# UM-ARM-Lab/pytorch_volumetric

Measured on AMD Instinct MI355X. Metric: SDF (val+grad) queries/sec, higher is better.
Workload: dtype f32

## Files before the change

### pytorch_volumetric_amd/csrc/composed.hip

```cpp
#include "common.h"
#include "grid_lookup.h"
#include "wave_ops.h"
#include "morton.h"

namespace pvamd {

constexpr int kUnnormalised = 1 << 30;
struct Best {
    float v, gx, gy, gz;
    int tag;
};

enum IndexMode { kEstimate = 0, kInlineExact = 1, kExact = 2 };

template <int MODE>
PVAMD_DEV void leaf_candidate(const pvamd_grid_t& g, const float* __restrict__ M, float px, float py, float pz,
                               float& v, float& a, float& b, float& c, uint64_t& vmask, bool& unsure) {
    const float x = affine_row(M[0], M[1], M[2], M[3], px, py, pz);
    const float y = affine_row(M[4], M[5], M[6], M[7], px, py, pz);
    const float z = affine_row(M[8], M[9], M[10], M[11], px, py, pz);
    vmask = in_range_mask(g, x, y, z);
    const bool valid = __builtin_amdgcn_inverse_ballot_w64(vmask);
    auto gather = [&]() {
        int flat;
// ... 901 lines not shown
    constexpr int N = NW * kTilePoints;
    __shared__ __attribute__((aligned(16))) float res[NW][1024];
    __shared__ float cull[kMaxCullLeaves][8];
    const int lane = threadIdx.x & 63, wave = __builtin_amdgcn_readfirstlane(threadIdx.x >> 6);
    const int a = a0 + blockIdx.x;
    build_cull_spheres(grids, S, tf, A, a, cull);
    __syncthreads();
    float scene = __builtin_inff();
    if (S <= kMaxCullLeaves) {
        float reach = -__builtin_inff();
        if (lane < S) {
            const float dx = cull[lane][0] - cull[0][0], dy = cull[lane][1] - cull[0][1], dz = cull[lane][2] - cull[0][2];
            reach = fast_sqrt(dx * dx + dy * dy + dz * dz) + cull[lane][3];
        }
        scene = wave_max(reach);
    }
    const float span = PVAMD_GROUP_MASK_SPAN * scene;
    for (int64_t chunk = blockIdx.y; chunk < nchunks; chunk += gridDim.y) {
        const int64_t cfirst = chunk * N <= P - N ? chunk * N : P - N;
        const int64_t run = chunk * N + wave * kTilePoints;
        const float* tb = bounds + 8 * (chunk * NW + wave);
        const float ct[3] = {tb[0], tb[1], tb[2]};
        const float rt = tb[3], mag = tb[4];
        float lower = -__builtin_inff();
        uint64_t todo = S >= 64 ? ~0ull : ((1ull << S) - 1ull);
        const bool masked = 2.f * rt <= span;
        if (masked) todo = leaf_mask_of_sphere(cull, S, lane, ct, rt, mag, lower);
        const GroupIO gio{sorted + 3 * run, perm + run, &res[0][0], cfirst, nullptr};
        if (masked) tile_passes_split<PPP, false, true, 1>(grids, S, tf, A, a, 0, P, val, leaf, nullptr, lane, todo, lower, gio);
        else tile_passes_split<PPP, false, false, 1>(grids, S, tf, A, a, 0, P, val, leaf, nullptr, lane, todo, lower, gio);
        __syncthreads();
        const f32x4_alias* sp = reinterpret_cast<const f32x4_alias*>(res[wave]);
        const int64_t o = (int64_t)a * P + cfirst + wave * kTilePoints;
        if constexpr (PACKED) {
            const float* rf = res[wave];
            f32x4* rec = reinterpret_cast<f32x4*>(val) + o;
#pragma unroll
            for (int k = 0; k < 4; ++k) {
                const int p = lane + 64 * k;
                rec[p] = f32x4{rf[768 + p], rf[3 * p], rf[3 * p + 1], rf[3 * p + 2]};
            }
        } else {
            __builtin_nontemporal_store(sp[192 + lane], reinterpret_cast<f32x4_u*>(val + o) + lane);
            f32x4_u* dst = reinterpret_cast<f32x4_u*>(grad + 3 * o);
            __builtin_nontemporal_store(sp[lane], dst + lane);
            __builtin_nontemporal_store(sp[lane + 64], dst + lane + 64);
            __builtin_nontemporal_store(sp[lane + 128], dst + lane + 128);
        }
        __syncthreads();
    }
}


template <int NW, int PPP>
__global__ __launch_bounds__(NW * 64, PVAMD_GROUP_MINWAVES) void composed_query_fused(
    const pvamd_grid_t* __restrict__ grids, int S, const float* __restrict__ tf, int A, const float* __restrict__ pts, int64_t nchunks,
    int64_t P, float* __restrict__ val, float* __restrict__ grad, int* __restrict__ leaf, int a0) {
    constexpr int N = NW * kTilePoints, kBins = N < 4096 ? N : 4096, kPerThread = kBins / (NW * 64), kKeyShift = kBins == 4096 ? 0 : (kBins == 2048 ? 1 : 2);
    static_assert(kBins >= 1024 && kBins % (NW * 64) == 0, "4, 8 or 16 waves");
    __shared__ __attribute__((aligned(16))) float res[NW][1024];
    __shared__ uint16_t sperm[N];
    __shared__ unsigned box[6];
    __shared__ unsigned wsum[NW];
    __shared__ __attribute__((aligned(16))) float wspan[NW];
    const int lane = threadIdx.x & 63, wave = __builtin_amdgcn_readfirstlane(threadIdx.x >> 6);
    const int a = a0 + blockIdx.x;
    auto hist = [&](int bin) -> unsigned& { return reinterpret_cast<unsigned*>(res[bin >> 8])[768 + (bin & 255)]; };
    for (int64_t chunk = blockIdx.y; chunk < nchunks; chunk += gridDim.y) {
        const int64_t cfirst = chunk * N <= P - N ? chunk * N : P - N;
        f32x4_alias* sp = reinterpret_cast<f32x4_alias*>(res[wave]);
        {
            const f32x4_u* src = reinterpret_cast<const f32x4_u*>(pts + 3 * (cfirst + wave * kTilePoints));
            sp[lane] = src[lane];
            sp[lane + 64] = src[lane + 64];
            sp[lane + 128] = src[lane + 128];
        }
        for (int i = threadIdx.x; i < kBins; i += NW * 64) hist(i) = 0u;
        if (threadIdx.x < 3) {
            box[threadIdx.x] = 0xffffffffu;
            box[3 + threadIdx.x] = 0u;
        }
        PVAMD_WAVE_SYNC();
        const f32x4 q0 = sp[3 * lane], q1 = sp[3 * lane + 1], q2 = sp[3 * lane + 2];
        const float px[4] = {q0.x, q0.w, q1.z, q2.y}, py[4] = {q0.y, q1.x, q1.w, q2.z}, pz[4] = {q0.z, q1.y, q2.x, q2.w};
        float lo[3], hi[3];
#pragma unroll
        for (int d = 0; d < 3; ++d) {
            lo[d] = __builtin_inff();
            hi[d] = -__builtin_inff();
        }
#pragma unroll
        for (int k = 0; k < 4; ++k) {
            const float c[3] = {px[k], py[k], pz[k]};
#pragma unroll
            for (int d = 0; d < 3; ++d) {
                const bool fin = fabsf(c[d]) < __builtin_inff();
                lo[d] = fin ? fminf(lo[d], c[d]) : lo[d];
                hi[d] = fin ? fmaxf(hi[d], c[d]) : hi[d];
            }
        }
        __syncthreads();
        float tile_span = 0.f;
#pragma unroll
        for (int d = 0; d < 3; ++d) {
            const float l = wave_min(lo[d]), h = wave_max(hi[d]);
            tile_span += fmaxf(h - l, 0.f);
            if (lane == 0) {
                atomicMin(&box[d], order_code(l));
                atomicMax(&box[3 + d], order_code(h));
            }
        }
        if (lane == 0) wspan[wave] = tile_span;
        __syncthreads();
        float blo[3], scale[3], chunk_span = 0.f;
#pragma unroll
        for (int d = 0; d < 3; ++d) {
            blo[d] = order_decode(box[d]);
            const float ext = order_decode(box[3 + d]) - blo[d];
            chunk_span += fmaxf(ext, 0.f);
            scale[d] = 15.999f / fmaxf(ext, 1e-30f);
        }
        float worst_tile = 0.f;
        if constexpr (NW % 4 == 0) {
            const f32x4_alias* w4 = reinterpret_cast<const f32x4_alias*>(wspan);
#pragma unroll
            for (int w = 0; w < NW / 4; ++w) {
                const f32x4 v = w4[w];
                worst_tile = fmaxf(worst_tile, fmaxf(fmaxf(v.x, v.y), fmaxf(v.z, v.w)));
            }
        } else {
            for (int w = 0; w < NW; ++w) worst_tile = fmaxf(worst_tile, wspan[w]);
        }
        const bool coherent = worst_tile <= kCoherentSpan * chunk_span;
        if (coherent) {
#pragma unroll
            for (int k = 0; k < 4; ++k) sperm[wave * kTilePoints + 4 * lane + k] = (uint16_t)(wave * kTilePoints + 4 * lane + k);
            PVAMD_WAVE_SYNC();
        } else {
        unsigned key[4], rank[4];
#pragma unroll
        for (int k = 0; k < 4; ++k) {
            key[k] = hilbert_cell16(px[k], py[k], pz[k], blo, scale) >> kKeyShift;
            rank[k] = atomicAdd(&hist((int)key[k]), 1u);
        }
        __syncthreads();
        unsigned local[kPerThread], sum = 0u;
#pragma unroll
        for (int i = 0; i < kPerThread; ++i) {
            local[i] = hist((int)threadIdx.x * kPerThread + i);
            sum += local[i];
        }
        unsigned inc = sum;
#pragma unroll
        for (int off = 1; off < 64; off <<= 1) {
            const unsigned t = __shfl_up(inc, off);
            inc += lane >= off ? t : 0u;
        }
        if (lane == 63) wsum[wave] = inc;
        __syncthreads();
        unsigned base = inc - sum;
        for (int w = 0; w < wave; ++w) base += wsum[w];
#pragma unroll
        for (int i = 0; i < kPerThread; ++i) {
            hist((int)threadIdx.x * kPerThread + i) = base;
            base += local[i];
        }
        __syncthreads();
#pragma unroll
        for (int k = 0; k < 4; ++k) sperm[hist((int)key[k]) + rank[k]] = (uint16_t)(wave * kTilePoints + 4 * lane + k);
        __syncthreads();
        }
        const GroupIO gio{nullptr, nullptr, &res[0][0], cfirst, sperm + wave * kTilePoints};
        const uint64_t todo = S >= 64 ? ~0ull : ((1ull << S) - 1ull);
        tile_passes_split<PPP, false, false, 2>(grids, S, tf, A, a, 0, P, val, leaf, nullptr, lane, todo, -__builtin_inff(), gio);
        __syncthreads();
        const int64_t o = (int64_t)a * P + cfirst + wave * kTilePoints;
        __builtin_nontemporal_store(sp[192 + lane], reinterpret_cast<f32x4_u*>(val + o) + lane);
        f32x4_u* dst = reinterpret_cast<f32x4_u*>(grad + 3 * o);
        __builtin_nontemporal_store(sp[lane], dst + lane);
        __builtin_nontemporal_store(sp[lane + 64], dst + lane + 64);
        __builtin_nontemporal_store(sp[lane + 128], dst + lane + 128);
        __syncthreads();
    }
}

}

using namespace pvamd;

static inline bool legacy_leaf_loop(int32_t flags, int32_t S) { return (flags & PVAMD_COMPOSED_LEGACY_LEAF_LOOP) || S >= kNoLeaf; }

extern "C" int pvamd_composed_query_packed(const pvamd_grid_t* grids, int32_t S, const float* tf, int32_t A,
                                           const float* points, int64_t Pp, float* out_rec, int32_t flags, void* stream) {
    if (S < 1 || A < 1 || Pp < 1 || Pp % kTilePoints != 0 || S >= kUnnormalised) return PVAMD_E_SHAPE;
    if (!grids || !tf || !points || !out_rec) return PVAMD_E_NULL;
    if (!aligned_to(grids, 8) || !aligned_to(tf, 4) || !aligned_to(points, 16) || !aligned_to(out_rec, 16)) return PVAMD_E_ALIGN;
    hipStream_t s = (hipStream_t)stream;
    const int64_t ntiles = Pp / kTilePoints;
    const int64_t tile_blocks = (ntiles + kWavesPerBlock - 1) / kWavesPerBlock;
    if (tile_blocks > 65535) return PVAMD_E_SHAPE;
    if (flags & PVAMD_COMPOSED_INLINE_EXACT)
        hipLaunchKernelGGL((composed_query_wave<PVAMD_COMPOSED_PPP, kInlineExact, true, 0>), dim3(A, (unsigned)tile_blocks),
                           dim3(kWavesPerBlock * 64), 0, s, grids, S, tf, A, points, ntiles, Pp, out_rec, nullptr, nullptr, 0);
    else if (legacy_leaf_loop(flags, S))
        hipLaunchKernelGGL((composed_query_wave<PVAMD_COMPOSED_PPP, kEstimate, true, 0>), dim3(A, (unsigned)tile_blocks),
                           dim3(kWavesPerBlock * 64), 0, s, grids, S, tf, A, points, ntiles, Pp, out_rec, nullptr, nullptr, 0);
    else
        hipLaunchKernelGGL((composed_query_wave<PVAMD_COMPOSED_PPP, kEstimate, true, 1>), dim3(A, (unsigned)tile_blocks),
                           dim3(kWavesPerBlock * 64), 0, s, grids, S, tf, A, points, ntiles, Pp, out_rec, nullptr, nullptr, 0);
    return (int)hipGetLastError();
}

extern "C" int pvamd_unpack_records(const float* rec, const int32_t* index, int64_t P, int64_t stride, int32_t A,
                                    float* out_val, float* out_grad, void* stream) {
    if (A < 1 || P < 1 || stride < 1) return PVAMD_E_SHAPE;
    if (!rec || !index || !out_val || !out_grad) return PVAMD_E_NULL;
    if (!aligned_to(rec, 16) || !aligned_to(index, 4) || !aligned_to(out_val, 4) || !aligned_to(out_grad, 4)) return PVAMD_E_ALIGN;
    const int64_t ntiles = (P + kTilePoints - 1) / kTilePoints;
    const int64_t tile_blocks = (ntiles + kUnpermuteWaves - 1) / kUnpermuteWaves;
    const int64_t groups = ((int64_t)A + 7) / 8;
    const int64_t ublocks = (tile_blocks + kUnpermuteTiles - 1) / kUnpermuteTiles;
    const int64_t blocks = groups * 8 * ublocks;
// ... 148 lines not shown
```

### pytorch_volumetric_amd/csrc/mesh.hip

```cpp
#include <cstdlib>
#include "common.h"
#include "mesh_math.h"
#include "morton.h"
#include "order_small.h"
#include "wave_ops.h"

namespace pvamd {

constexpr int kRec = PVAMD_TRI_REC;
constexpr int kTile = PVAMD_TRI_TILE;
constexpr int kGroup = PVAMD_TRI_GROUP;
constexpr int kGroupsPerTile = kTile / kGroup;
static_assert(kTile == 256 && kGroup == 16 && kRec == 24, "the scan is written for 256-record tiles of six float4 planes");
enum { kPlaneSphere = 0, kPlaneU = 1, kPlaneV = 2, kPlaneA = 3, kPlaneB = 4, kPlaneC = 5 };
constexpr int kTileFloats = kTile * kRec;
PVAMD_DEV const f32x4* tile_plane(const float* rec, int tile, int plane) {
    return reinterpret_cast<const f32x4*>(rec + (int64_t)tile * kTileFloats + plane * (kTile * 4));
}
PVAMD_DEV f32x4 record_plane(const float* rec, int j, int plane) { return tile_plane(rec, j / kTile, plane)[j % kTile]; }

struct MeshArgs {
    const float* normal;
    const float* rec;
    const float* tiles;
// ... 158 lines not shown
    const float du = fmaxf(fabsf(u) - hu, 0.f), dv = fmaxf(fabsf(v) - hv, 0.f);
    const float lb2 = fmaf(dv, dv, fmaf(du, du, h2));
    return !(lb2 > fmaf(8e-6f, dist2, s.reach2m + m0));
}

#ifdef PVAMD_MESH_STATS
__device__ unsigned long long g_stats[32];
__device__ long long g_nested;
#define STAT(i, v) do { if ((threadIdx.x & 63) == 0) atomicAdd(&g_stats[i], (unsigned long long)(v)); } while (0)
extern "C" int pvamd_debug_stats(unsigned long long* out, int reset) {
    (void)hipMemcpyFromSymbol(out, HIP_SYMBOL(g_stats), sizeof(g_stats));
    if (reset) { unsigned long long z[32] = {}; (void)hipMemcpyToSymbol(HIP_SYMBOL(g_stats), z, sizeof(z)); }
    return 0;
}
#define TIC(t) const long long t = __builtin_readcyclecounter()
#define TOC(i, t) STAT(i, __builtin_readcyclecounter() - t)
#define TOC_NET(i, t, inner) STAT(i, __builtin_readcyclecounter() - t - (inner))
#else
#define STAT(i, v)
#define TIC(t)
#define TOC(i, t)
#define TOC_NET(i, t, inner)
#endif

constexpr int kQueueCap = 128;
constexpr unsigned long long kBestInit = 0x7F80000000000000ull;

template <bool WITH_RAY>
struct WaveLocal {
    f32x4 sphere[64], fu[64], fv[64];
    float m0[64];
    unsigned qc[kQueueCap];
    unsigned qr[WITH_RAY ? kQueueCap : 1];
};
template <bool WITH_RAY>
struct GroupShared {
    unsigned long long best[64];
    int hits[WITH_RAY ? 64 : 1];
    int handed;
    float dir[WITH_RAY ? 192 : 1];
    float dn[WITH_RAY ? 192 : 1];
};
template <int SLICES, bool WITH_RAY>
struct MeshShared {
    GroupShared<WITH_RAY> g;
    WaveLocal<WITH_RAY> w[SLICES];
};

PVAMD_DEV float uniform(float v) { return __int_as_float(__builtin_amdgcn_readfirstlane(__float_as_int(v))); }
PVAMD_DEV V3 xyz(f32x4 v) { return v3(v.x, v.y, v.z); }

struct WaveBound {
    LaneState q;
    float rho;
    V3 dn0;
    float k, rho_k;
};

template <bool WITH_RAY>
struct Wave {
    LaneState s;
    bool live;
    V3 dn, dir;
    WaveBound wb;
    int nc, nr;
};

template <bool WITH_RAY>
PVAMD_DEV void refresh_bound(Wave<WITH_RAY>& wv) {
    const float rmax = wave_max(wv.live ? wv.s.reach : 0.f);
    set_reach(wv.wb.q, uniform((rmax + wv.wb.rho) * 1.00001f));
}

template <bool WITH_RAY>
PVAMD_DEV void pull_reach(const GroupShared<WITH_RAY>& g, Wave<WITH_RAY>& wv) {
    const float d2 = __int_as_float((int)(unsigned)(g.best[threadIdx.x & 63] >> 32));
    const float reach = fast_sqrt(d2) * 1.00001f + 1.1e-19f;
    if (reach < wv.s.reach) set_reach(wv.s, reach);
    refresh_bound(wv);
}

template <bool WITH_RAY>
PVAMD_DEV bool wave_setup(const MeshArgs& m, Wave<WITH_RAY>& wv) {
    const V3 p = wv.s.p;
    wv.live = fabsf(p.x) < INFINITY && fabsf(p.y) < INFINITY && fabsf(p.z) < INFINITY;
    wv.nc = wv.nr = 0;
    set_reach(wv.s, INFINITY);
    if (__ballot(wv.live) == 0ull) return false;
    const float lx = wave_min(wv.live ? p.x : INFINITY), hx = wave_max(wv.live ? p.x : -INFINITY);
    const float ly = wave_min(wv.live ? p.y : INFINITY), hy = wave_max(wv.live ? p.y : -INFINITY);
    const float lz = wave_min(wv.live ? p.z : INFINITY), hz = wave_max(wv.live ? p.z : -INFINITY);
    wv.wb.q.p = v3(uniform(0.5f * lx + 0.5f * hx), uniform(0.5f * ly + 0.5f * hy), uniform(0.5f * lz + 0.5f * hz));
    const V3 d = v3(p.x - wv.wb.q.p.x, p.y - wv.wb.q.p.y, p.z - wv.wb.q.p.z);
    wv.wb.rho = uniform(wave_max(wv.live ? fast_sqrt(dot(d, d)) : 0.f) * 1.00001f + 1.1e-19f);
    wv.wb.dn0 = v3(0.f, 0.f, 0.f);
    wv.wb.k = wv.wb.rho_k = 0.f;
    if (WITH_RAY) {
        const V3 a = v3((float)m.ray_dir[0], (float)m.ray_dir[1], (float)m.ray_dir[2]);
        const float inv = 1.f / sqrt_rn(dot(a, a));
        wv.wb.dn0 = v3(uniform(a.x * inv), uniform(a.y * inv), uniform(a.z * inv));
        const V3 e = v3(wv.dn.x - wv.wb.dn0.x, wv.dn.y - wv.wb.dn0.y, wv.dn.z - wv.wb.dn0.z);
        const float chord = wave_max(wv.live ? fast_sqrt(dot(e, e)) : 0.f);
        wv.wb.k = uniform(2.001f * chord + 2e-6f);
        wv.wb.rho_k = uniform(wv.wb.rho * (1.f + wv.wb.k) * 1.00001f);
    }
    set_reach(wv.wb.q, INFINITY);
    return true;
}

PVAMD_DEV bool axis_may_hit(const WaveBound& wb, V3 w, float dist2, float r) {
    const float dist = fast_sqrt(dist2) * 1.00001f + 1.1e-19f;
    return sphere_may_hit(dist2, dot(w, wb.dn0), fmaf(wb.k, dist, r + wb.rho_k));
}

PVAMD_DEV void enqueue(unsigned* q, int& n, unsigned long long mask, bool mine, int j) {
    const int lane = threadIdx.x & 63;
    if (mine) q[n + __popcll(mask & ((1ull << lane) - 1ull))] = ((unsigned)j << 6) | (unsigned)lane;
    n += __popcll(mask);
}

template <class Fn>
PVAMD_DEV void drain(unsigned* q, int& n, bool everything, Fn&& fn) {
    const int lane = threadIdx.x & 63;
    PVAMD_WAVE_SYNC();
    STAT(6, 1);
    fn(n < 64 ? n : 64, q);
    if (n > 64) {
        const int rem = n - 64;
        if (everything) {
            STAT(6, 1);
            fn(rem, q + 64);
            n = 0;
        } else {
            const unsigned v = lane < rem ? q[64 + lane] : 0u;
            if (lane < rem) q[lane] = v;
            n = rem;
        }
    } else {
        n = 0;
    }
    PVAMD_WAVE_SYNC();
}

template <bool WITH_RAY>
PVAMD_DEV void drain_closest(const MeshArgs& m, GroupShared<WITH_RAY>& g, WaveLocal<WITH_RAY>& wl, Wave<WITH_RAY>& wv, bool everything) {
    if (wv.nc == 0) return;
    const int lane = threadIdx.x & 63;
    TIC(t_drain);
    drain(wl.qc, wv.nc, everything, [&](int count, const unsigned* q) {
        PVAMD_COUNT_PAIRS(m, 0, count);
        const unsigned e = lane < count ? q[lane] : 0u;
        const int owner = e & 63;
        const V3 p = v3(__shfl(wv.s.p.x, owner, 64), __shfl(wv.s.p.y, owner, 64), __shfl(wv.s.p.z, owner, 64));
        if (lane < count) {
            const int j = (int)(e >> 6);
            const f32x4 A = record_plane(m.rec, j, kPlaneA), B = record_plane(m.rec, j, kPlaneB), C = record_plane(m.rec, j, kPlaneC);
            const V3 qp = sub(closest_point_triangle(p, xyz(A), xyz(B), xyz(C)), p);
            const float d2 = dot(qp, qp);
            atomicMin(&g.best[owner], ((unsigned long long)(unsigned)__float_as_int(d2) << 32) | (unsigned)__float_as_int(A.w));
        }
    });
    pull_reach(g, wv);
    TOC(16, t_drain);
}

template <bool WITH_RAY>
PVAMD_DEV void drain_rays(const MeshArgs& m, GroupShared<WITH_RAY>& g, WaveLocal<WITH_RAY>& wl, Wave<WITH_RAY>& wv, bool everything) {
    if (wv.nr == 0) return;
    const int lane = threadIdx.x & 63;
    drain(wl.qr, wv.nr, everything, [&](int count, const unsigned* q) {
        PVAMD_COUNT_PAIRS(m, 1, count);
        const unsigned e = lane < count ? q[lane] : 0u;
        const int owner = e & 63;
        const V3 p = v3(__shfl(wv.s.p.x, owner, 64), __shfl(wv.s.p.y, owner, 64), __shfl(wv.s.p.z, owner, 64));
        const V3 d = v3(__shfl(wv.dir.x, owner, 64), __shfl(wv.dir.y, owner, 64), __shfl(wv.dir.z, owner, 64));
        if (lane < count) {
            const int j = (int)(e >> 6);
            const f32x4 A = record_plane(m.rec, j, kPlaneA), B = record_plane(m.rec, j, kPlaneB), C = record_plane(m.rec, j, kPlaneC);
            if (ray_hits_triangle(p, d, xyz(A), xyz(B), xyz(C))) atomicAdd(&g.hits[owner], 1);
        }
    });
}

template <bool WITH_RAY>
PVAMD_DEV void visit_tile(const MeshArgs& m, GroupShared<WITH_RAY>& g, WaveLocal<WITH_RAY>& wl, Wave<WITH_RAY>& wv, int ti,
                          int pass_lo = 0, int pass_hi = kTile / 64) {
    const int lane = threadIdx.x & 63;
    const int ntiles = (m.F + kTile - 1) / kTile;
    const int n = min(kTile, m.F - ti * kTile);
    STAT(1, 1);
    TIC(t_visit);
    unsigned gm = 0u;
#ifdef PVAMD_MESH_STATS
    unsigned mine_groups = 0u;
#endif
    {
        const bool gv = lane < kGroupsPerTile && lane * kGroup < n;
        const f32x4 gs = reinterpret_cast<const f32x4*>(m.tiles)[ntiles + ti * kGroupsPerTile + (gv ? lane : 0)];
        const V3 wc = v3(gs.x - wv.wb.q.p.x, gs.y - wv.wb.q.p.y, gs.z - wv.wb.q.p.z);
        const float dc2 = dot(wc, wc);
        bool coarse = sphere_may_improve(wv.wb.q, dc2, gs.w);
        if (WITH_RAY) coarse = coarse || axis_may_hit(wv.wb, wc, dc2, gs.w);
        unsigned todo = (unsigned)__ballot(coarse && gv);
        todo &= ((1u << (pass_hi * (64 / kGroup))) - 1u) & ~((1u << (pass_lo * (64 / kGroup))) - 1u);
        while (todo != 0u) {
            const int b = __builtin_ctz(todo);
            todo &= todo - 1u;
            const V3 ctr = v3(__int_as_float(__builtin_amdgcn_readlane(__float_as_int(gs.x), b)),
                              __int_as_float(__builtin_amdgcn_readlane(__float_as_int(gs.y), b)),
                              __int_as_float(__builtin_amdgcn_readlane(__float_as_int(gs.z), b)));
            const float r = __int_as_float(__builtin_amdgcn_readlane(__float_as_int(gs.w), b));
            const V3 w = v3(ctr.x - wv.s.p.x, ctr.y - wv.s.p.y, ctr.z - wv.s.p.z);
            const float dist2 = dot(w, w);
            bool need = sphere_may_improve(wv.s, dist2, r);
            if (WITH_RAY) need = need || sphere_may_hit(dist2, dot(w, wv.dn), r);
            STAT(9, 1);
#ifdef PVAMD_MESH_STATS
            if (need && wv.live) mine_groups |= 1u << b;
#endif
            if (__ballot(need && wv.live) != 0ull) gm |= 1u << b;
        }
    }
    const f32x4* P0 = tile_plane(m.rec, ti, kPlaneSphere);
    const f32x4* P1 = tile_plane(m.rec, ti, kPlaneU);
    const f32x4* P2 = tile_plane(m.rec, ti, kPlaneV);
    const f32x4* P4 = tile_plane(m.rec, ti, kPlaneB);
    for (int pass = pass_lo; pass < pass_hi; ++pass) {
        if (((gm >> (pass * (64 / kGroup))) & ((1u << (64 / kGroup)) - 1u)) == 0u) continue;
        STAT(2, 1);
#ifdef PVAMD_MESH_STATS
        {
            const int st_points = __popcll(__ballot(((mine_groups >> (pass * (64 / kGroup))) & 0xFu) != 0u));
            STAT(22, st_points);
        }
#endif
        const int idx = pass * 64 + lane;
        const f32x4 a0 = P0[idx], a1 = P1[idx], a2 = P2[idx];
        const float am0 = P4[idx].w;
        bool keep_c, keep_r = false;
        {
            const bool valid = idx < n && ((gm >> (idx / kGroup)) & 1u);
            const V3 w = v3(a0.x - wv.wb.q.p.x, a0.y - wv.wb.q.p.y, a0.z - wv.wb.q.p.z);
            const float dist2 = dot(w, w);
            keep_c = valid && sphere_may_improve(wv.wb.q, dist2, a0.w) &&
                     rect_may_improve(wv.wb.q, w, dist2, xyz(a1), a1.w, xyz(a2), a2.w, am0);
            if (WITH_RAY) keep_r = valid && axis_may_hit(wv.wb, w, dist2, a0.w);
        }
        const unsigned long long mc = __ballot(keep_c), mr = WITH_RAY ? __ballot(keep_r) : 0ull;
        unsigned long long todo = mc | mr;
        if (todo == 0ull) continue;
        PVAMD_WAVE_SYNC();
        wl.sphere[lane] = a0;
        wl.fu[lane] = a1;
        wl.fv[lane] = a2;
        wl.m0[lane] = am0;
        PVAMD_WAVE_SYNC();
        const int j0 = ti * kTile + pass * 64;
        const unsigned long long live_mask = __ballot(wv.live);
        TIC(t_surv);
        while (todo != 0ull) {
            const int b = __builtin_ctzll(todo);
            todo &= todo - 1ull;
            STAT(3, 1);
            const f32x4 o = wl.sphere[b];
            const V3 w = v3(o.x - wv.s.p.x, o.y - wv.s.p.y, o.z - wv.s.p.z);
            const float dist2 = dot(w, w);
            if (!WITH_RAY || ((mc >> b) & 1ull)) {
                const unsigned long long near_c = live_mask & __ballot(sphere_may_improve(wv.s, dist2, o.w));
                if (near_c != 0ull) {
                    STAT(7, 1);
                    const f32x4 u = wl.fu[b], v = wl.fv[b];
                    const unsigned long long mk = near_c & __ballot(rect_may_improve(wv.s, w, dist2, xyz(u), u.w, xyz(v), v.w, wl.m0[b]));
                    if (mk) {
                        STAT(4, __popcll(mk)); STAT(8, 1);
                        enqueue(wl.qc, wv.nc, mk, __builtin_amdgcn_inverse_ballot_w64(mk), j0 + b);
                        if (wv.nc >= 64) drain_closest(m, g, wl, wv, false);
                    }
                }
            }
            if (WITH_RAY && ((mr >> b) & 1ull)) {
                const unsigned long long mk = live_mask & __ballot(sphere_may_hit(dist2, dot(w, wv.dn), o.w));
                if (mk) {
                    STAT(5, __popcll(mk)); STAT(8, 1);
                    enqueue(wl.qr, wv.nr, mk, __builtin_amdgcn_inverse_ballot_w64(mk), j0 + b);
                    if (wv.nr >= 64) drain_rays(m, g, wl, wv, false);
                }
            }
        }
        TOC(18, t_surv);
    }
    TOC(17, t_visit);
}

template <bool WITH_RAY>
PVAMD_DEV int scan_seed(const MeshArgs& m, Wave<WITH_RAY>& wv, int part, int nparts) {
    const int lane = threadIdx.x & 63;
    const int ntiles = (m.F + kTile - 1) / kTile;
    const f32x4* tiles4 = reinterpret_cast<const f32x4*>(m.tiles);
// ... 9 lines not shown
            if ((nparts == 1 || (ti % nparts) == part) && (b < own || nearest < 0)) {
                own = b < own ? b : own;
                nearest = ti;
            }
        }
    }
    const float lowest = wave_min(bound);
    set_reach(wv.s, (lowest + wv.wb.rho) * 1.00001f);
    refresh_bound(wv);
    const float mine = wave_min(own);
    unsigned long long at = __ballot(nearest >= 0 && own == mine);
    if (at == 0ull) at = __ballot(nearest >= 0);
    return at ? __builtin_amdgcn_readlane(nearest, __builtin_ctzll(at)) : -1;
}

template <bool WITH_RAY>
PVAMD_DEV void greedy_reach(const MeshArgs& m, GroupShared<WITH_RAY>& g, Wave<WITH_RAY>& wv, int ti) {
    const int ntiles = (m.F + kTile - 1) / kTile;
    const f32x4* spheres = reinterpret_cast<const f32x4*>(m.tiles);
    const V3 p = wv.s.p;
    auto reach_of = [&](f32x4 sp) {
        const V3 w = v3(sp.x - p.x, sp.y - p.y, sp.z - p.z);
        return fast_sqrt(dot(w, w)) * 1.00001f + (sp.w + 1.1e-19f);
    };
    float bound = INFINITY;
    int gi = 0;
    const int ngroups = (min(kTile, m.F - ti * kTile) + kGroup - 1) / kGroup;
    for (int k = 0; k < ngroups; ++k) {
        const float b = reach_of(spheres[ntiles + ti * kGroupsPerTile + k]);
        if (b < bound) { bound = b; gi = k; }
    }
    const int j0 = ti * kTile + gi * kGroup;
    float nearest = INFINITY;
    int jn = -1;
    for (int k = 0; k < kGroup; ++k) {
        if (j0 + k < m.F) {
            const float b = reach_of(record_plane(m.rec, j0 + k, kPlaneSphere));
            if (b < nearest) { nearest = b; jn = j0 + k; }
        }
    }
#ifndef PVAMD_MESH_NO_GREEDY_EXACT
    PVAMD_COUNT_PAIRS(m, 0, __popcll(__ballot(jn >= 0 && wv.live)));
    if (jn >= 0 && wv.live) {
        const f32x4 A = record_plane(m.rec, jn, kPlaneA), B = record_plane(m.rec, jn, kPlaneB), C = record_plane(m.rec, jn, kPlaneC);
        const V3 qp = sub(closest_point_triangle(p, xyz(A), xyz(B), xyz(C)), p);
        const float d2 = dot(qp, qp);
        atomicMin(&g.best[threadIdx.x & 63], ((unsigned long long)(unsigned)__float_as_int(d2) << 32) | (unsigned)__float_as_int(A.w));
        STAT(4, 1);
    }
#endif
    bound = fminf(bound, nearest) * 1.00001f;
    if (bound < wv.s.reach) set_reach(wv.s, bound);
    pull_reach(g, wv);
}

template <bool WITH_RAY>
PVAMD_DEV void scan_tiles(const MeshArgs& m, GroupShared<WITH_RAY>& g, WaveLocal<WITH_RAY>& wl, Wave<WITH_RAY>& wv, int skip,
                          int part, int nparts, int pass_lo = 0, int pass_hi = kTile / 64) {
    const int lane = threadIdx.x & 63;
    const int ntiles = (m.F + kTile - 1) / kTile;
    const f32x4* tiles4 = reinterpret_cast<const f32x4*>(m.tiles);
    for (int base = 0; base < ntiles; base += 64) {
        const int ti = base + lane;
        const bool mine = ti < ntiles && ti != skip && (nparts == 1 || (ti % nparts) == part);
        const f32x4 ts = tiles4[mine ? ti : 0];
        const V3 w = v3(ts.x - wv.wb.q.p.x, ts.y - wv.wb.q.p.y, ts.z - wv.wb.q.p.z);
        const float dist2 = dot(w, w);
        const bool ray = WITH_RAY && mine && axis_may_hit(wv.wb, w, dist2, ts.w);
        STAT(0, 1);
        const float lower = mine ? fast_sqrt(dist2) - ts.w : INFINITY;
        unsigned long long done = 0ull;
        for (;;) {
            pull_reach(g, wv);
            const bool need = mine && (ray || sphere_may_improve(wv.wb.q, dist2, ts.w));
            const unsigned long long todo = __ballot(need) & ~done;
            if (todo == 0ull) break;
            const float key = ((todo >> lane) & 1ull) ? lower : INFINITY;
            const unsigned long long at = __ballot(key == wave_min(key)) & todo;
            const int t = __builtin_ctzll(at ? at : todo);
            done |= 1ull << t;
            const V3 ctr = v3(__int_as_float(__builtin_amdgcn_readlane(__float_as_int(ts.x), t)),
                              __int_as_float(__builtin_amdgcn_readlane(__float_as_int(ts.y), t)),
                              __int_as_float(__builtin_amdgcn_readlane(__float_as_int(ts.z), t)));
            const float r = __int_as_float(__builtin_amdgcn_readlane(__float_as_int(ts.w), t));
            const V3 wl_ = v3(ctr.x - wv.s.p.x, ctr.y - wv.s.p.y, ctr.z - wv.s.p.z);
            const float d2 = dot(wl_, wl_);
            bool mine_too = sphere_may_improve(wv.s, d2, r);
            if (WITH_RAY) mine_too = mine_too || sphere_may_hit(d2, dot(wl_, wv.dn), r);
            if (__ballot(mine_too && wv.live) == 0ull) continue;
            visit_tile<WITH_RAY>(m, g, wl, wv, base + t, pass_lo, pass_hi);
        }
    }
}

template <bool WITH_RAY>
PVAMD_DEV void scan_finish(const MeshArgs& m, GroupShared<WITH_RAY>& g, WaveLocal<WITH_RAY>& wl, Wave<WITH_RAY>& wv) {
    drain_closest(m, g, wl, wv, true);
    if (WITH_RAY) drain_rays(m, g, wl, wv, true);
}

template <bool WITH_RAY>
PVAMD_DEV bool scan_begin(const MeshArgs& m, GroupShared<WITH_RAY>& g, Wave<WITH_RAY>& wv, int wave, uint64_t seed,
                          int64_t jitter_index, const unsigned long long* start, const float* __restrict__ drawn = nullptr,
                          const float* __restrict__ bound = nullptr) {
    const int lane = threadIdx.x & 63;
    if (wave == 0) {
        g.best[lane] = start ? *start : kBestInit;
        if (WITH_RAY) {
            g.hits[lane] = 0;
            const V3 dir = drawn ? v3(drawn[3 * lane], drawn[3 * lane + 1], drawn[3 * lane + 2])
                                 : jitter_dir(m.ray_dir, seed, jitter_index);
            const float inv_len = 1.f / sqrt_rn(dot(dir, dir));
            g.dir[3 * lane] = dir.x; g.dir[3 * lane + 1] = dir.y; g.dir[3 * lane + 2] = dir.z;
            g.dn[3 * lane] = dir.x * inv_len; g.dn[3 * lane + 1] = dir.y * inv_len; g.dn[3 * lane + 2] = dir.z * inv_len;
        }
    }
    __syncthreads();
    wv.dir = wv.dn = v3(0.f, 0.f, 0.f);
    if (WITH_RAY) {
        wv.dir = v3(g.dir[3 * lane], g.dir[3 * lane + 1], g.dir[3 * lane + 2]);
        wv.dn = v3(g.dn[3 * lane], g.dn[3 * lane + 1], g.dn[3 * lane + 2]);
    }
    return bound ? load_bound(bound, wv) : wave_setup(m, wv);
}

struct HandOver {
    int* count;
// ... 35 lines not shown
#endif
#ifndef PVAMD_MESH_HEAVY_PARTS
#define PVAMD_MESH_HEAVY_PARTS 32
#endif
constexpr int kHeavy32nds = PVAMD_MESH_HEAVY_32NDS;
#ifndef PVAMD_MESH_HEAVY_MIN_TILES
#define PVAMD_MESH_HEAVY_MIN_TILES 128
#endif
constexpr int kHeavyMinTiles = PVAMD_MESH_HEAVY_MIN_TILES;
constexpr int kHeavyParts = PVAMD_MESH_HEAVY_PARTS;

PVAMD_DEV void store_bound(float* __restrict__ b, const WaveBound& wb, bool any_live) {
    if ((threadIdx.x & 63) != 0) return;
    b[0] = wb.q.p.x; b[1] = wb.q.p.y; b[2] = wb.q.p.z; b[3] = wb.rho;
    b[4] = wb.dn0.x; b[5] = wb.dn0.y; b[6] = wb.dn0.z; b[7] = wb.k;
    b[8] = wb.rho_k; b[9] = any_live ? 1.f : 0.f;
    b[10] = wb.q.reach;
}
template <bool WITH_RAY>
PVAMD_DEV bool part_has_work(const MeshArgs& m, const float* __restrict__ b, int part, int nparts) {
    if (uniform(b[9]) == 0.f) return false;
    WaveBound wb;
    wb.q.p = v3(uniform(b[0]), uniform(b[1]), uniform(b[2]));
    wb.rho = uniform(b[3]);
    wb.dn0 = v3(uniform(b[4]), uniform(b[5]), uniform(b[6]));
    wb.k = uniform(b[7]);
    wb.rho_k = uniform(b[8]);
    set_reach(wb.q, uniform(b[10]));
    const int lane = threadIdx.x & 63;
    const int ntiles = (m.F + kTile - 1) / kTile;
    const f32x4* tiles4 = reinterpret_cast<const f32x4*>(m.tiles);
    for (int base = part; base < ntiles; base += 64 * nparts) {
        const int ti = base + lane * nparts;
        const f32x4 ts = tiles4[ti < ntiles ? ti : 0];
        const V3 w = v3(ts.x - wb.q.p.x, ts.y - wb.q.p.y, ts.z - wb.q.p.z);
        const float dist2 = dot(w, w);
        bool need = sphere_may_improve(wb.q, dist2, ts.w);
        if (WITH_RAY) need = need || axis_may_hit(wb, w, dist2, ts.w);
        if (__ballot(need && ti < ntiles) != 0ull) return true;
    }
    return false;
}
template <bool WITH_RAY>
PVAMD_DEV bool load_bound(const float* __restrict__ b, Wave<WITH_RAY>& wv) {
    const V3 p = wv.s.p;
    wv.live = fabsf(p.x) < INFINITY && fabsf(p.y) < INFINITY && fabsf(p.z) < INFINITY;
    wv.nc = wv.nr = 0;
    set_reach(wv.s, INFINITY);
    wv.wb.q.p = v3(uniform(b[0]), uniform(b[1]), uniform(b[2]));
    wv.wb.rho = uniform(b[3]);
    wv.wb.dn0 = v3(uniform(b[4]), uniform(b[5]), uniform(b[6]));
    wv.wb.k = uniform(b[7]);
    wv.wb.rho_k = uniform(b[8]);
    set_reach(wv.wb.q, INFINITY);
    return uniform(b[9]) != 0.f;
}

template <bool WITH_RAY>
PVAMD_DEV int flagged_tiles(const MeshArgs& m, const Wave<WITH_RAY>& wv) {
    const int lane = threadIdx.x & 63;
    const int ntiles = (m.F + kTile - 1) / kTile;
    const f32x4* tiles4 = reinterpret_cast<const f32x4*>(m.tiles);
    int n = 0;
    for (int base = 0; base < ntiles; base += 64) {
        const int ti = base + lane;
        const f32x4 ts = tiles4[ti < ntiles ? ti : 0];
        const V3 w = v3(ts.x - wv.wb.q.p.x, ts.y - wv.wb.q.p.y, ts.z - wv.wb.q.p.z);
        const float dist2 = dot(w, w);
        bool need = sphere_may_improve(wv.wb.q, dist2, ts.w);
        if (WITH_RAY) need = need || axis_may_hit(wv.wb, w, dist2, ts.w);
        n += __popcll(__ballot(need && ti < ntiles));
    }
    return n;
}

template <int SLICES, bool WITH_RAY>
PVAMD_DEV bool scan_mesh(const MeshArgs& m, MeshShared<SLICES, WITH_RAY>& sh, Wave<WITH_RAY>& wv, int wave, uint64_t seed,
                         int64_t jitter_index, const HandOver& ho, int group, int transform) {
    const int lane = threadIdx.x & 63;
    bool handed = false;
    TIC(t_all);
    if (scan_begin(m, sh.g, wv, wave, seed, jitter_index, nullptr) && m.F > 0) {
        TIC(t_seed);
        const int first = scan_seed(m, wv, wave, SLICES);
        if (first >= 0) {
#ifndef PVAMD_MESH_NO_GREEDY
            greedy_reach(m, sh.g, wv, first);
#endif
            TOC(20, t_seed);
            visit_tile<WITH_RAY>(m, sh.g, sh.w[wave], wv, first);
            drain_closest(m, sh.g, sh.w[wave], wv, true);
        }
        if (ho.cap > 0 && (m.F + kTile - 1) / kTile >= kHeavyMinTiles) {
            __syncthreads();
            if (wave == 0) {
                pull_reach(sh.g, wv);
                int slot = -1;
                if (flagged_tiles(m, wv) * 32 >= ((m.F + kTile - 1) / kTile) * kHeavy32nds) {
                    if (lane == 0) slot = atomicAdd(ho.count, 1);
                    slot = __builtin_amdgcn_readfirstlane(slot);
                    if (slot >= ho.cap) slot = -1;
                }
                if (slot >= 0) {
                    if (lane == 0) {
                        ho.entries[2 * slot] = group;
                        ho.entries[2 * slot + 1] = transform;
// ... 266 lines not shown

__global__ __launch_bounds__(64) void hand_over_gather_kernel(MeshArgs m, const int* __restrict__ order, const float* __restrict__ pts,
                                                              int64_t P, HandOver ho, int groups) {
    const int g = blockIdx.x, lane = threadIdx.x;
    const int64_t slot = (int64_t)g * 64 + lane;
    const int64_t i = point_index(order, slot, P);
    const V3 dir = v3(ho.p_dir[3 * i], ho.p_dir[3 * i + 1], ho.p_dir[3 * i + 2]);
    const float reach = ho.p_reach[i];
    ho.best[slot] = ho.p_best[i];
    ho.reach[slot] = reach;
    ho.hits[slot] = 0;
    float* o = ho.dir + slot * 3;
    o[0] = dir.x; o[1] = dir.y; o[2] = dir.z;
    Wave<true> wv{};
    wv.s.p = v3(pts[3 * i], pts[3 * i + 1], pts[3 * i + 2]);
    float* q = ho.pts + slot * 3;
    q[0] = wv.s.p.x; q[1] = wv.s.p.y; q[2] = wv.s.p.z;
    const float inv_len = 1.f / sqrt_rn(dot(dir, dir));
    wv.dir = dir;
    wv.dn = v3(dir.x * inv_len, dir.y * inv_len, dir.z * inv_len);
    const bool any_live = wave_setup(m, wv);
    if (any_live) {
        set_reach(wv.s, reach);
        refresh_bound(wv);
    }
    store_bound(ho.bound + (int64_t)g * kBoundFloats, wv.wb, any_live);
    if (lane == 0) {
        ho.entries[2 * g] = g;
        ho.entries[2 * g + 1] = 0;
        if (g == 0) *ho.count = groups;
    }
}

#ifndef PVAMD_MESH_PARTS_WAVES
#define PVAMD_MESH_PARTS_WAVES 7
#endif
template <bool WITH_RAY, bool WAIT = false, int WAVES = kTile / 64>
PVAMD_DEV void parts_of_group(const MeshArgs& m, MeshShared<WAVES, WITH_RAY>& sh, const int* __restrict__ order,
                              const float* __restrict__ M, const float* __restrict__ pts, int64_t P, uint64_t seed,
                              int64_t index_base, const HandOver& ho, int slot, int group) {
    const int lane = threadIdx.x & 63, wave = __builtin_amdgcn_readfirstlane(threadIdx.x >> 6);
    if (!part_has_work<WITH_RAY>(m, ho.bound + (int64_t)slot * kBoundFloats, (int)blockIdx.y, (int)gridDim.y)) return;
    Wave<WITH_RAY> wv;
    const float* q = ho.pts + ((int64_t)slot * 64 + lane) * 3;
    wv.s.p = v3(q[0], q[1], q[2]);
    const unsigned long long start = ho.best[(int64_t)slot * 64 + lane];
    const float known = ho.reach[(int64_t)slot * 64 + lane];
    TIC(t_parts);
    if (scan_begin(m, sh.g, wv, wave, seed, 0, &start, WITH_RAY ? ho.dir + (int64_t)slot * 192 : nullptr,
                   ho.bound + (int64_t)slot * kBoundFloats)) {
        if (__any(wv.live && !(known < INFINITY) && (unsigned)(start >> 32) >= 0x7F800000u)) scan_seed(m, wv, 0, 1);
        if (known < wv.s.reach) set_reach(wv.s, known);
        refresh_bound(wv);
        constexpr int kPasses = (kTile / 64) / WAVES;
        scan_tiles<WITH_RAY>(m, sh.g, sh.w[wave], wv, -1, (int)blockIdx.y, (int)gridDim.y, wave * kPasses, (wave + 1) * kPasses);
        scan_finish(m, sh.g, sh.w[wave], wv);
    }
    TOC(21, t_parts);
    __syncthreads();
    if (wave == 0) {
        if (WAIT) {
            unsigned long long was = 0ull;
            int had = 0;
            if (sh.g.best[lane] < start) was = atomicMin(&ho.best[(int64_t)slot * 64 + lane], sh.g.best[lane]);
            if (WITH_RAY && sh.g.hits[lane] != 0) had = atomicAdd(&ho.hits[(int64_t)slot * 64 + lane], sh.g.hits[lane]);
            asm volatile("" ::"v"(was), "v"(had) : "memory");
        } else {
            if (sh.g.best[lane] < start) atomicMin(&ho.best[(int64_t)slot * 64 + lane], sh.g.best[lane]);
            if (WITH_RAY && sh.g.hits[lane] != 0) atomicAdd(&ho.hits[(int64_t)slot * 64 + lane], sh.g.hits[lane]);
        }
    }
}

template <int kAllWaves>
__global__ __launch_bounds__(64 * kAllWaves, PVAMD_MESH_PARTS_WAVES) void mesh_parts_all_kernel(MeshArgs m, const int* __restrict__ order,
                                                                          const float* __restrict__ pts, int64_t P,
                                                                          uint64_t seed, int64_t index_base, HandOver ho, QueryOut out) {
    __shared__ __attribute__((aligned(16))) MeshShared<kAllWaves, true> sh;
    const int g = (int)blockIdx.x;
    parts_of_group<true, true, kAllWaves>(m, sh, order, nullptr, pts, P, seed, index_base, ho, g, g);
    if (threadIdx.x >= 64) return;
    const int lane = threadIdx.x;
    int done = 0;
    if (lane == 0) done = atomicAdd(&ho.entries[2 * g + 1], 1);
    if (__builtin_amdgcn_readfirstlane(done) != (int)gridDim.y - 1) return;
    const int64_t k = (int64_t)g * 64 + lane;
    if (k >= P) return;
    const int64_t i = order ? (int64_t)order[k] : k;
    const unsigned long long found = atomicMin(&ho.best[k], ~0ull);
    const int hits = atomicOr(&ho.hits[k], 0);
    write_query(m, out, i, v3(pts[3 * i], pts[3 * i + 1], pts[3 * i + 2]), found, hits);
}

template <bool WITH_RAY, int WAVES>
__global__ __launch_bounds__(64 * WAVES, PVAMD_MESH_PARTS_WAVES) void mesh_parts_kernel(MeshArgs m, const int* __restrict__ order,
                                                                      const float* __restrict__ W,
                                                                      const float* __restrict__ pts, int64_t P,
                                                                      uint64_t seed, int64_t index_base, HandOver ho) {
    __shared__ __attribute__((aligned(16))) MeshShared<WAVES, WITH_RAY> sh;
    const int listed = min(*ho.count, ho.cap);
    for (int slot = blockIdx.x; slot < listed; slot += gridDim.x) {
        parts_of_group<WITH_RAY, false, WAVES>(m, sh, order, W ? W + 16 * (int64_t)ho.entries[2 * slot + 1] : nullptr, pts, P, seed, index_base,
                                 ho, slot, ho.entries[2 * slot]);
        __syncthreads();
    }
}
// ... 351 lines not shown
```

Baseline: 203.6 billion.

## Shrink fused-kernel sort histogram and replace block scans with wave-local DPP scan

Reduces the Hilbert-key histogram in the fused composed query kernel to a small configurable bin count (default 512) held in its own shared array. Every wave now computes the exclusive prefix redundantly with a DPP inclusive scan, which removes the cross-wave scan, its two block barriers and the per-wave sum array. The chunk bounding box is reduced from per-wave slots with group reductions instead of shared atomics, which also drops one barrier. In exchange the Hilbert ordering is coarser, so the sort may give less spatial coherence for grid lookups. The bin starts are also packed as uint16 into each wave's scratch area.

```diff
diff --git a/pytorch_volumetric_amd/csrc/composed.hip b/pytorch_volumetric_amd/csrc/composed.hip
--- a/pytorch_volumetric_amd/csrc/composed.hip
+++ b/pytorch_volumetric_amd/csrc/composed.hip
@@ -977,20 +977,37 @@
 }
 
 
+#ifndef PVAMD_FUSED_BINS
+#define PVAMD_FUSED_BINS 512
+#endif
+constexpr int kFusedBins = PVAMD_FUSED_BINS;
+typedef unsigned u32_alias __attribute__((may_alias));
+typedef uint16_t u16_alias __attribute__((may_alias));
+
+PVAMD_DEV unsigned wave_inclusive_sum(unsigned v) {
+    v += (unsigned)__builtin_amdgcn_update_dpp(0, (int)v, 0x111, 0xf, 0xf, false);
+    v += (unsigned)__builtin_amdgcn_update_dpp(0, (int)v, 0x112, 0xf, 0xf, false);
+    v += (unsigned)__builtin_amdgcn_update_dpp(0, (int)v, 0x114, 0xf, 0xf, false);
+    v += (unsigned)__builtin_amdgcn_update_dpp(0, (int)v, 0x118, 0xf, 0xf, false);
+    v += (unsigned)__builtin_amdgcn_update_dpp(0, (int)v, 0x142, 0xa, 0xf, false);
+    v += (unsigned)__builtin_amdgcn_update_dpp(0, (int)v, 0x143, 0xc, 0xf, false);
+    return v;
+}
+
 template <int NW, int PPP>
 __global__ __launch_bounds__(NW * 64, PVAMD_GROUP_MINWAVES) void composed_query_fused(
     const pvamd_grid_t* __restrict__ grids, int S, const float* __restrict__ tf, int A, const float* __restrict__ pts, int64_t nchunks,
     int64_t P, float* __restrict__ val, float* __restrict__ grad, int* __restrict__ leaf, int a0) {
-    constexpr int N = NW * kTilePoints, kBins = N < 4096 ? N : 4096, kPerThread = kBins / (NW * 64), kKeyShift = kBins == 4096 ? 0 : (kBins == 2048 ? 1 : 2);
-    static_assert(kBins >= 1024 && kBins % (NW * 64) == 0, "4, 8 or 16 waves");
+    constexpr int N = NW * kTilePoints, kBins = kFusedBins, kPerLane = kBins / 64;
+    constexpr int kKeyShift = kBins == 512 ? 3 : (kBins == 256 ? 4 : (kBins == 128 ? 5 : 6));
+    static_assert(kBins == 512 || kBins == 256 || kBins == 128 || kBins == 64, "a wave's uint16 bin starts fill at most its 1 KB value quarter");
+    static_assert(NW <= 16 && (NW & (NW - 1)) == 0 && N <= 65535, "a row of 16 lanes folds the wave boxes; positions are uint16");
     __shared__ __attribute__((aligned(16))) float res[NW][1024];
     __shared__ uint16_t sperm[N];
-    __shared__ unsigned box[6];
-    __shared__ unsigned wsum[NW];
-    __shared__ __attribute__((aligned(16))) float wspan[NW];
+    __shared__ __attribute__((aligned(16))) unsigned hist[kBins];
+    __shared__ float wbox[7][NW];
     const int lane = threadIdx.x & 63, wave = __builtin_amdgcn_readfirstlane(threadIdx.x >> 6);
     const int a = a0 + blockIdx.x;
-    auto hist = [&](int bin) -> unsigned& { return reinterpret_cast<unsigned*>(res[bin >> 8])[768 + (bin & 255)]; };
     for (int64_t chunk = blockIdx.y; chunk < nchunks; chunk += gridDim.y) {
         const int64_t cfirst = chunk * N <= P - N ? chunk * N : P - N;
         f32x4_alias* sp = reinterpret_cast<f32x4_alias*>(res[wave]);
@@ -1000,11 +1017,7 @@
             sp[lane + 64] = src[lane + 64];
             sp[lane + 128] = src[lane + 128];
         }
-        for (int i = threadIdx.x; i < kBins; i += NW * 64) hist(i) = 0u;
-        if (threadIdx.x < 3) {
-            box[threadIdx.x] = 0xffffffffu;
-            box[3 + threadIdx.x] = 0u;
-        }
+        for (int i = threadIdx.x; i < kBins; i += NW * 64) hist[i] = 0u;
         PVAMD_WAVE_SYNC();
         const f32x4 q0 = sp[3 * lane], q1 = sp[3 * lane + 1], q2 = sp[3 * lane + 2];
         const float px[4] = {q0.x, q0.w, q1.z, q2.y}, py[4] = {q0.y, q1.x, q1.w, q2.z}, pz[4] = {q0.z, q1.y, q2.x, q2.w};
@@ -1024,38 +1037,27 @@
                 hi[d] = fin ? fmaxf(hi[d], c[d]) : hi[d];
             }
         }
-        __syncthreads();
         float tile_span = 0.f;
 #pragma unroll
         for (int d = 0; d < 3; ++d) {
             const float l = wave_min(lo[d]), h = wave_max(hi[d]);
             tile_span += fmaxf(h - l, 0.f);
             if (lane == 0) {
-                atomicMin(&box[d], order_code(l));
-                atomicMax(&box[3 + d], order_code(h));
-            }
-        }
-        if (lane == 0) wspan[wave] = tile_span;
+                wbox[d][wave] = l;
+                wbox[3 + d][wave] = h;
+            }
+        }
+        if (lane == 0) wbox[6][wave] = tile_span;
         __syncthreads();
         float blo[3], scale[3], chunk_span = 0.f;
 #pragma unroll
         for (int d = 0; d < 3; ++d) {
-            blo[d] = order_decode(box[d]);
-            const float ext = order_decode(box[3 + d]) - blo[d];
+            blo[d] = group16_min(wbox[d][lane & (NW - 1)]);
+            const float ext = group16_max(wbox[3 + d][lane & (NW - 1)]) - blo[d];
             chunk_span += fmaxf(ext, 0.f);
             scale[d] = 15.999f / fmaxf(ext, 1e-30f);
         }
-        float worst_tile = 0.f;
-        if constexpr (NW % 4 == 0) {
-            const f32x4_alias* w4 = reinterpret_cast<const f32x4_alias*>(wspan);
-#pragma unroll
-            for (int w = 0; w < NW / 4; ++w) {
-                const f32x4 v = w4[w];
-                worst_tile = fmaxf(worst_tile, fmaxf(fmaxf(v.x, v.y), fmaxf(v.z, v.w)));
-            }
-        } else {
-            for (int w = 0; w < NW; ++w) worst_tile = fmaxf(worst_tile, wspan[w]);
-        }
+        const float worst_tile = group16_max(wbox[6][lane & (NW - 1)]);
         const bool coherent = worst_tile <= kCoherentSpan * chunk_span;
         if (coherent) {
 #pragma unroll
@@ -1066,33 +1068,31 @@
 #pragma unroll
         for (int k = 0; k < 4; ++k) {
             key[k] = hilbert_cell16(px[k], py[k], pz[k], blo, scale) >> kKeyShift;
-            rank[k] = atomicAdd(&hist((int)key[k]), 1u);
+            rank[k] = atomicAdd(&hist[key[k]], 1u);
         }
         __syncthreads();
-        unsigned local[kPerThread], sum = 0u;
-#pragma unroll
-        for (int i = 0; i < kPerThread; ++i) {
-            local[i] = hist((int)threadIdx.x * kPerThread + i);
+        unsigned local[kPerLane], sum = 0u;
+#pragma unroll
+        for (int i = 0; i < kPerLane; ++i) {
+            local[i] = hist[lane * kPerLane + i];
             sum += local[i];
         }
-        unsigned inc = sum;
-#pragma unroll
-        for (int off = 1; off < 64; off <<= 1) {
-            const unsigned t = __shfl_up(inc, off);
-            inc += lane >= off ? t : 0u;
-        }
-        if (lane == 63) wsum[wave] = inc;
-        __syncthreads();
-        unsigned base = inc - sum;
-        for (int w = 0; w < wave; ++w) base += wsum[w];
-#pragma unroll
-        for (int i = 0; i < kPerThread; ++i) {
-            hist((int)threadIdx.x * kPerThread + i) = base;
-            base += local[i];
-        }
-        __syncthreads();
-#pragma unroll
-        for (int k = 0; k < 4; ++k) sperm[hist((int)key[k]) + rank[k]] = (uint16_t)(wave * kTilePoints + 4 * lane + k);
+        unsigned base = wave_inclusive_sum(sum) - sum;
+        u32_alias* mine = reinterpret_cast<u32_alias*>(res[wave] + 768);
+        if constexpr (kPerLane == 1) {
+            reinterpret_cast<u16_alias*>(mine)[lane] = (uint16_t)base;
+        } else {
+#pragma unroll
+            for (int i = 0; i < kPerLane; i += 2) {
+                const unsigned second = base + local[i];
+                mine[lane * (kPerLane / 2) + i / 2] = base | (second << 16);
+                base = second + local[i + 1];
+            }
+        }
+        PVAMD_WAVE_SYNC();
+        const u16_alias* start = reinterpret_cast<const u16_alias*>(mine);
+#pragma unroll
+        for (int k = 0; k < 4; ++k) sperm[start[key[k]] + rank[k]] = (uint16_t)(wave * kTilePoints + 4 * lane + k);
         __syncthreads();
         }
         const GroupIO gio{nullptr, nullptr, &res[0][0], cfirst, sperm + wave * kTilePoints};
```

New measurement: 204.2 billion, median of 2. About the same (+0.3%).

## Add second far-center bounding sphere to cull mesh tiles and records

Applied to the files above, without the earlier changes.

Adds a second wave-uniform culling sphere, placed opposite the nearest known triangle relative to the wave center. It bounds every lane's search ball from another direction, and intersecting it with the existing wave sphere lets the scan reject more groups, tiles and records. The cost is extra per-candidate distance tests and wave reductions, plus more registers, which could lower occupancy. The far sphere is built after seeding and after hand-over start values.

```diff
diff --git a/pytorch_volumetric_amd/csrc/mesh.hip b/pytorch_volumetric_amd/csrc/mesh.hip
--- a/pytorch_volumetric_amd/csrc/mesh.hip
+++ b/pytorch_volumetric_amd/csrc/mesh.hip
@@ -234,6 +234,8 @@
 
 struct WaveBound {
     LaneState q;
+    LaneState far;
+    bool far_on;
     float rho;
     V3 dn0;
     float k, rho_k;
@@ -245,6 +247,7 @@
     bool live;
     V3 dn, dir;
     WaveBound wb;
+    float far_dist;
     int nc, nr;
 };
 
@@ -252,6 +255,37 @@
 PVAMD_DEV void refresh_bound(Wave<WITH_RAY>& wv) {
     const float rmax = wave_max(wv.live ? wv.s.reach : 0.f);
     set_reach(wv.wb.q, uniform((rmax + wv.wb.rho) * 1.00001f));
+    if (wv.wb.far_on) {
+        const float fmax = wave_max(wv.live ? wv.far_dist + wv.s.reach : 0.f);
+        set_reach(wv.wb.far, uniform(fmax * 1.00001f));
+    }
+}
+
+PVAMD_DEV bool far_may_improve(const WaveBound& wb, V3 ctr, float r) {
+    if (!wb.far_on) return true;
+    const V3 w = sub(ctr, wb.far.p);
+    return sphere_may_improve(wb.far, dot(w, w), r);
+}
+
+PVAMD_DEV int nearest_lane(float key, bool valid) {
+    const float k = valid ? key : INFINITY;
+    const unsigned long long at = __ballot(valid && k == wave_min(k));
+    return at ? (int)__builtin_ctzll(at) : -1;
+}
+
+constexpr float kFarLambda = 1.f;
+template <bool WITH_RAY>
+PVAMD_DEV void choose_far(Wave<WITH_RAY>& wv, V3 toward) {
+    const V3 c = wv.wb.q.p;
+    const V3 d = sub(toward, c);
+    const float s = kFarLambda * wv.wb.q.reach / fast_sqrt(dot(d, d));
+    const V3 cf = v3(uniform(c.x - s * d.x), uniform(c.y - s * d.y), uniform(c.z - s * d.z));
+    if (!(fabsf(cf.x) < INFINITY && fabsf(cf.y) < INFINITY && fabsf(cf.z) < INFINITY)) return;
+    wv.wb.far.p = cf;
+    wv.wb.far_on = true;
+    const V3 e = sub(wv.s.p, cf);
+    wv.far_dist = fast_sqrt(dot(e, e)) * 1.00001f + 1.1e-19f;
+    refresh_bound(wv);
 }
 
 template <bool WITH_RAY>
@@ -268,6 +302,7 @@
     wv.live = fabsf(p.x) < INFINITY && fabsf(p.y) < INFINITY && fabsf(p.z) < INFINITY;
     wv.nc = wv.nr = 0;
     set_reach(wv.s, INFINITY);
+    wv.far_dist = INFINITY;
     if (__ballot(wv.live) == 0ull) return false;
     const float lx = wave_min(wv.live ? p.x : INFINITY), hx = wave_max(wv.live ? p.x : -INFINITY);
     const float ly = wave_min(wv.live ? p.y : INFINITY), hy = wave_max(wv.live ? p.y : -INFINITY);
@@ -286,6 +321,9 @@
         wv.wb.k = uniform(2.001f * chord + 2e-6f);
         wv.wb.rho_k = uniform(wv.wb.rho * (1.f + wv.wb.k) * 1.00001f);
     }
+    wv.wb.far.p = wv.wb.q.p;
+    wv.wb.far_on = false;
+    set_reach(wv.wb.far, INFINITY);
     set_reach(wv.wb.q, INFINITY);
     return true;
 }
@@ -381,7 +419,7 @@
         const f32x4 gs = reinterpret_cast<const f32x4*>(m.tiles)[ntiles + ti * kGroupsPerTile + (gv ? lane : 0)];
         const V3 wc = v3(gs.x - wv.wb.q.p.x, gs.y - wv.wb.q.p.y, gs.z - wv.wb.q.p.z);
         const float dc2 = dot(wc, wc);
-        bool coarse = sphere_may_improve(wv.wb.q, dc2, gs.w);
+        bool coarse = sphere_may_improve(wv.wb.q, dc2, gs.w) && far_may_improve(wv.wb, xyz(gs), gs.w);
         if (WITH_RAY) coarse = coarse || axis_may_hit(wv.wb, wc, dc2, gs.w);
         unsigned todo = (unsigned)__ballot(coarse && gv);
         todo &= ((1u << (pass_hi * (64 / kGroup))) - 1u) & ~((1u << (pass_lo * (64 / kGroup))) - 1u);
@@ -426,6 +464,12 @@
             const float dist2 = dot(w, w);
             keep_c = valid && sphere_may_improve(wv.wb.q, dist2, a0.w) &&
                      rect_may_improve(wv.wb.q, w, dist2, xyz(a1), a1.w, xyz(a2), a2.w, am0);
+            if (wv.wb.far_on) {
+                const V3 wf = sub(xyz(a0), wv.wb.far.p);
+                const float distf2 = dot(wf, wf);
+                keep_c = keep_c && sphere_may_improve(wv.wb.far, distf2, a0.w) &&
+                         rect_may_improve(wv.wb.far, wf, distf2, xyz(a1), a1.w, xyz(a2), a2.w, am0);
+            }
             if (WITH_RAY) keep_r = valid && axis_may_hit(wv.wb, w, dist2, a0.w);
         }
         const unsigned long long mc = __ballot(keep_c), mr = WITH_RAY ? __ballot(keep_r) : 0ull;
@@ -541,6 +585,8 @@
     bound = fminf(bound, nearest) * 1.00001f;
     if (bound < wv.s.reach) set_reach(wv.s, bound);
     pull_reach(g, wv);
+    const int l = nearest_lane(wv.s.reach, wv.live && jn >= 0);
+    if (l >= 0) choose_far(wv, xyz(record_plane(m.rec, __builtin_amdgcn_readlane(jn, l), kPlaneSphere)));
 }
 
 template <bool WITH_RAY>
@@ -561,7 +607,7 @@
         unsigned long long done = 0ull;
         for (;;) {
             pull_reach(g, wv);
-            const bool need = mine && (ray || sphere_may_improve(wv.wb.q, dist2, ts.w));
+            const bool need = mine && (ray || (sphere_may_improve(wv.wb.q, dist2, ts.w) && far_may_improve(wv.wb, xyz(ts), ts.w)));
             const unsigned long long todo = __ballot(need) & ~done;
             if (todo == 0ull) break;
             const float key = ((todo >> lane) & 1ull) ? lower : INFINITY;
@@ -703,6 +749,10 @@
     wv.wb.dn0 = v3(uniform(b[4]), uniform(b[5]), uniform(b[6]));
     wv.wb.k = uniform(b[7]);
     wv.wb.rho_k = uniform(b[8]);
+    wv.wb.far.p = wv.wb.q.p;
+    wv.wb.far_on = false;
+    set_reach(wv.wb.far, INFINITY);
+    wv.far_dist = INFINITY;
     set_reach(wv.wb.q, INFINITY);
     return uniform(b[9]) != 0.f;
 }
@@ -1075,6 +1125,10 @@
         if (__any(wv.live && !(known < INFINITY) && (unsigned)(start >> 32) >= 0x7F800000u)) scan_seed(m, wv, 0, 1);
         if (known < wv.s.reach) set_reach(wv.s, known);
         refresh_bound(wv);
+        if (!WAIT) {
+            const int l = nearest_lane(__int_as_float((int)(unsigned)(start >> 32)), wv.live && (unsigned)(start >> 32) < 0x7F800000u);
+            if (l >= 0) choose_far(wv, xyz(record_plane(m.rec, m.rec_of_face[__builtin_amdgcn_readlane((int)(unsigned)start, l)], kPlaneSphere)));
+        }
         constexpr int kPasses = (kTile / 64) / WAVES;
         scan_tiles<WITH_RAY>(m, sh.g, sh.w[wave], wv, -1, (int)blockIdx.y, (int)gridDim.y, wave * kPasses, (wave + 1) * kPasses);
         scan_finish(m, sh.g, sh.w[wave], wv);
```

Result: no change. 201.2 billion before, 204.3 billion after (median of 2 runs) (+1.5%).
